# qiskit-community/adapt-aqc

Hardware: AMD Instinct MI355X
Metric: overlap+gradient evals/sec, 50-qubit MPS chi=64, 1/2/4/8 MI355X (higher is better)
Workload: dtype c128

## Files before the change

adaptaqc_amd/_lib.py:

```python
import atexit
import ctypes
import os
import threading

import numpy as np

_HERE = os.path.dirname(os.path.abspath(__file__))
LIB_PATH = os.environ.get("AQC_LIB") or os.path.join(_HERE, "libaqchip.so")

OP_DTYPE = np.dtype(
    [("nq", "<i4"), ("q0", "<i4"), ("q1", "<i4"), ("flags", "<i4"), ("m", "<f8", (32,))], align=True
)
assert OP_DTYPE.itemsize == 272
OP_KRAUS1 = 1
OP_MEASURE1 = 2
OP_KRAUS2 = 3

EXPORTS = (
    "aqc_last_error", "aqc_version", "aqc_init", "aqc_finalize", "aqc_timing_enable",
    "aqc_timing_query", "aqc_timing_reset",
    "aqc_sv_create", "aqc_sv_destroy", "aqc_sv_reset", "aqc_sv_copy", "aqc_sv_apply", "aqc_sv_plan",
    "aqc_sv_amp0", "aqc_sv_z_all", "aqc_sv_get", "aqc_sv_set",
    "aqc_mps_create", "aqc_mps_destroy", "aqc_mps_set_truncation", "aqc_mps_set_vidal",
    "aqc_mps_get_vidal", "aqc_mps_get_dims", "aqc_mps_copy", "aqc_mps_copy_batch", "aqc_mps_apply",
    "aqc_mps_apply_batch", "aqc_mps_apply_sort_batch", "aqc_mps_apply_sort_batch_async", "aqc_mps_apply_batch_async", "aqc_mps_check_batch", "aqc_mps_sort", "aqc_mps_sort_batch", "aqc_mps_overlap_zero",
    "aqc_mps_overlap_zero_batch", "aqc_mps_dot", "aqc_mps_z_all", "aqc_mps_amps_hw1", "aqc_mps_z_all_batch", "aqc_mps_z_sum_batch", "aqc_mps_zero_hw1_batch",
    "aqc_mps_amps_hw1_batch",
    "aqc_pair_grads", "aqc_pair_grads_batch", "aqc_argmax_scaled", "aqc_argmax_scaled_batch", "aqc_mps_jacobi_stats",
    "aqc_mps_set_jacobi_tol", "aqc_mps_set_jacobi_stop", "aqc_mps_set_fused_chain", "aqc_mps_chain_ticks", "aqc_svd_debug",
    "aqc_sv_pair_rdms", "aqc_mps_pair_rdms", "aqc_mps_pair_rdms_batch", "aqc_entanglement_measures",
    "aqc_sv_transition", "aqc_mps_product_fit", "aqc_mps_set_svd_path", "aqc_svd_gram_ticks", "aqc_bj_ticks",
    "aqc_sweep_set_chain_mode", "aqc_stream_join", "aqc_stream_wait", "aqc_svd_gram_stats", "aqc_env_ticks",
    "aqc_comm_unique_id", "aqc_comm_init", "aqc_comm_destroy", "aqc_comm_rank", "aqc_allgather_f64",
    "aqc_allgather_f64_host", "aqc_allreduce_max_f64", "aqc_svd_gram_big_stats", "aqc_svd_gram_big_ticks",
    "aqc_gb_set_spin_limit", "aqc_gb_set_tail", "aqc_gb_set_stages", "aqc_debug_hog", "aqc_pool_stats",
    "aqc_scratch_stats",
    "aqc_env_fallbacks", "aqc_env_set_single", "aqc_env_set_spin_limit",
    "aqc_sv_sample", "aqc_mps_sample", "aqc_sample_uniforms", "aqc_sv_traj_sample",
    "aqc_sv_traj_pair_tomo", "aqc_sv_traj_pauli_counts", "aqc_mps_traj_sample", "aqc_mps_traj_plan", "aqc_mps_traj_set_batch",
    "aqc_mps_traj_pair_tomo", "aqc_mps_traj_tomo_plan", "aqc_mps_traj_set_readout_batch",
    "aqc_sv_pauli_expect", "aqc_mps_pauli_expect", "aqc_mps_pauli_expect_batch",
    "aqc_pair_tomo_probs", "aqc_concurrence_bound_probs", "aqc_multinomial_counts", "aqc_tomo_fit",
)


class AqcError(RuntimeError):
    pass


_lock = threading.Lock()
_lib = None
_initialised_device = None

_P = ctypes.c_void_p
_I = ctypes.c_int
_D = ctypes.c_double
_DP = ctypes.POINTER(ctypes.c_double)
_IP = ctypes.POINTER(ctypes.c_int)

_SIGS = {
    "aqc_last_error": ([], ctypes.c_char_p),
    "aqc_version": ([], _I),
    "aqc_init": ([_I], _I),
    "aqc_finalize": ([], _I),
    "aqc_timing_enable": ([_I], _I),
    "aqc_timing_query": ([ctypes.c_char_p, _DP, ctypes.POINTER(ctypes.c_int64), _DP, _DP], _I),
    "aqc_timing_reset": ([], _I),
    "aqc_sv_create": ([_I, ctypes.POINTER(_P)], _I),
    "aqc_sv_destroy": ([_P], _I),
# ... 9 lines not shown
    "aqc_mps_destroy": ([_P], _I),
    "aqc_mps_set_truncation": ([_P, _D, _I], _I),
    "aqc_mps_set_vidal": ([_P, _P, _P, _P], _I),
    "aqc_mps_get_vidal": ([_P, _P, _P, _P], _I),
    "aqc_mps_get_dims": ([_P, _P], _I),
    "aqc_mps_copy": ([_P, _P], _I),
    "aqc_mps_copy_batch": ([_P, _P, _I], _I),
    "aqc_mps_apply": ([_P, _P, _I], _I),
    "aqc_mps_apply_batch": ([_P, _I, _P, _P], _I),
    "aqc_mps_apply_sort_batch": ([_P, _I, _P, _P], _I),
    "aqc_mps_apply_sort_batch_async": ([_P, _I, _P, _P], _I),
    "aqc_mps_apply_batch_async": ([_P, _I, _P, _P], _I),
    "aqc_mps_check_batch": ([_P, _I], _I),
    "aqc_mps_sort": ([_P], _I),
    "aqc_mps_sort_batch": ([_P, _I], _I),
    "aqc_mps_overlap_zero": ([_P, _DP, _DP], _I),
    "aqc_mps_overlap_zero_batch": ([_P, _I, _P], _I),
    "aqc_mps_dot": ([_P, _P, _DP, _DP], _I),
    "aqc_mps_z_all": ([_P, _P], _I),
    "aqc_mps_amps_hw1": ([_P, _P], _I),
    "aqc_mps_z_all_batch": ([_P, _I, _P], _I),
    "aqc_mps_z_sum_batch": ([_P, _P, _I, _P], _I),
    "aqc_mps_zero_hw1_batch": ([_P, _P, _I, _P, _P], _I),
    "aqc_mps_amps_hw1_batch": ([_P, _I, _P], _I),
    "aqc_pair_grads": ([_P, _P, _P, _I, _P, _P, _P, _I, _P, _I], _I),
    "aqc_pair_grads_batch": ([_P, _I, _P, _P, _I, _P, _P, _P, _I, _P, _I], _I),
    "aqc_argmax_scaled": ([_P, _P, _I, _I, _IP], _I),
    "aqc_argmax_scaled_batch": ([_P, _I, _P, _I, _I, _P], _I),
    "aqc_mps_jacobi_stats": ([_P, _IP], _I),
    "aqc_mps_set_jacobi_tol": ([_D], _I),
    "aqc_mps_set_jacobi_stop": ([_D], _I),
    "aqc_mps_set_fused_chain": ([_I], _I),
    "aqc_mps_chain_ticks": ([_P], _I),
    "aqc_svd_debug": ([_P, _I, _I, _I, _I, _P, _P, _P, _P], _I),
    "aqc_sv_pair_rdms": ([_P, _P, _I, _P], _I),
    "aqc_mps_pair_rdms": ([_P, _P, _I, _P], _I),
    "aqc_mps_pair_rdms_batch": ([_P, _I, _P, _I, _P, _I], _I),
    "aqc_entanglement_measures": ([_P, _I, _I, _P, _I], _I),
    "aqc_sv_transition": ([_P, _P, _I, _P], _I),
    "aqc_mps_product_fit": ([_P, _P, _I, _I, _I, _D, _DP, _IP], _I),
    "aqc_mps_set_svd_path": ([_I, _I], _I),
    "aqc_svd_gram_ticks": ([_P], _I),
    "aqc_bj_ticks": ([_P], _I),
    "aqc_sweep_set_chain_mode": ([_I], _I),
    "aqc_stream_join": ([_P], _I),
    "aqc_stream_wait": ([_P], _I),
    "aqc_svd_gram_stats": ([_P], _I),
    "aqc_env_ticks": ([_P], _I),
    "aqc_comm_unique_id": ([ctypes.c_char_p], _I),
    "aqc_comm_init": ([ctypes.c_char_p, _I, _I, ctypes.POINTER(_P)], _I),
    "aqc_comm_destroy": ([_P], _I),
    "aqc_comm_rank": ([_P, _IP, _IP], _I),
    "aqc_allgather_f64": ([_P, _P, _P, ctypes.c_size_t], _I),
    "aqc_allgather_f64_host": ([_P, _P, _P, ctypes.c_size_t], _I),
    "aqc_allreduce_max_f64": ([_P, _DP], _I),
    "aqc_svd_gram_big_stats": ([_P], _I),
    "aqc_svd_gram_big_ticks": ([_P], _I),
    "aqc_gb_set_spin_limit": ([_D], _I),
    "aqc_env_fallbacks": ([ctypes.POINTER(ctypes.c_longlong)], _I),
    "aqc_env_set_single": ([_I], _I),
    "aqc_env_set_spin_limit": ([_D], _I),
    "aqc_gb_set_tail": ([_I], _I),
    "aqc_gb_set_stages": ([_I], _I),
    "aqc_debug_hog": ([_I, _D], _I),
    "aqc_pool_stats": ([_P], _I),
    "aqc_scratch_stats": ([_P], _I),
# ... 94 lines not shown
    arr["q0"] = np.fromiter((q[0] for _, q in ops), dtype=np.int32, count=n)
    arr["q1"] = np.fromiter((q[1] if len(q) == 2 else 0 for _, q in ops), dtype=np.int32, count=n)
    m = arr["m"]
    for k, width in ((1, 4), (2, 16)):
        idx = np.flatnonzero(nq == k)
        if idx.size:
            mats = np.asarray([ops[i][0] for i in idx], dtype=np.complex128).reshape(idx.size, width)
            m[idx, : 2 * width] = mats.view(np.float64)
    return arr


def timing_enable(on=True):
    check(load().aqc_timing_enable(1 if on else 0))


def timing_reset():
    check(load().aqc_timing_reset())


def timing_query(name):
    ms, b, f = ctypes.c_double(), ctypes.c_double(), ctypes.c_double()
    n = ctypes.c_int64()
    check(load().aqc_timing_query(name.encode(), ctypes.byref(ms), ctypes.byref(n), ctypes.byref(b), ctypes.byref(f)))
    return {"ms": ms.value, "launches": n.value, "bytes": b.value, "flops": f.value}


def gram_stats():
    out = np.zeros(6)
    check(load().aqc_svd_gram_stats(ptr(out)))
    return {"calls": int(out[0]), "taken": int(out[1]), "declined_shape": int(out[2]),
            "declined_floor": int(out[3]), "certificates": int(out[4]), "certified": int(out[5])}


def gram_big_stats():
    out = np.zeros(8)
    check(load().aqc_svd_gram_big_stats(ptr(out)))
    return {"calls": int(out[0]), "taken": int(out[1]), "declined": int(out[2]),
            "declined_floor": int(out[3]), "timeouts": int(out[4]), "certificates": int(out[5]),
            "certified": int(out[6]), "declined_certificate": int(out[7])}
```

adaptaqc_amd/csrc/mps.hip:

```cpp
#include <algorithm>
#include <cmath>
#include <chrono>
#include <cstring>
#include <atomic>
#include <cstdlib>
#include <mutex>
#include <thread>
#include <unordered_set>

#include "aqc_gemm.h"
#include "mps_internal.h"

using aqc::cplx;

namespace aqc {

namespace {
std::mutex g_mps_stream_mu;
hipStream_t g_mps_streams[64] = {nullptr};
void release_mps_streams() {
  std::lock_guard<std::mutex> lk(g_mps_stream_mu);
  for (auto& s : g_mps_streams)
    if (s) (void)hipStreamDestroy(s), s = nullptr;
}
// ... 10 lines not shown
  }
  return g_mps_streams[dev];
}

hipStream_t mps_stream_if_any(int dev) {
  if (dev < 0 || dev >= 64) return nullptr;
  std::lock_guard<std::mutex> lk(g_mps_stream_mu);
  return g_mps_streams[dev];
}

StagingRing& staging_ring() {
  static PerDevice<StagingRing> rings;
  return rings.here();
}

}

namespace {

using aqc::fresh_tid;
using aqc::StagingLease;
using aqc::wave_sum_d;

constexpr int kT = 256;
constexpr double kChop = 1e-16;
constexpr int kMaxSweeps = 60;
double g_jacobi_tol_factor = 1.0;
constexpr double kDefaultTinyT = 1e-6;
constexpr double kStopCos = 3e-13;
constexpr int kStopCosSweeps = 30;
double g_jacobi_tiny_t = kDefaultTinyT;
constexpr double kJacobiNoise = 0.0;
bool g_fused_chain = true;
int g_chain_min_states = 32;
constexpr int kChainLdsBytes = 4 * (int)sizeof(aqc::GemmLds);

struct OneSiteJob {
  cplx* g;
  const int* dims;
  int cap;
  int pad;
  cplx u[4];
};

using aqc::TwoSiteJob;
using aqc::kMaxCap;
using aqc::kSigMax;
using aqc::kSigTail;
using aqc::kSigLen;

__global__ void k_mps_zero(cplx* gam, double* lam, int* dims, int n, int cap) {
  const size_t ss = (size_t)2 * cap * cap;
  for (int i = blockIdx.x * blockDim.x + threadIdx.x; i < n; i += gridDim.x * blockDim.x) {
    gam[(size_t)i * ss] = aqc::cmk(1.0, 0.0);
  }
  for (int b = blockIdx.x * blockDim.x + threadIdx.x; b <= n; b += gridDim.x * blockDim.x) {
    lam[(size_t)b * cap] = 1.0;
    dims[b] = 1;
  }
}

__global__ __launch_bounds__(kT) void k_1q(const OneSiteJob* __restrict__ jobs) {
  const OneSiteJob& j = jobs[blockIdx.y];
  const int cl = j.dims[0], cr = j.dims[1];
  const int cap = j.cap;
  const size_t half = (size_t)cap * cap;
// ... 580 lines not shown
  __shared__ double norm_s;
  const int chl = j.dims[0], chr = j.dims[2];
  const int M = 2 * chl, N = 2 * chr;
  const int C = M < N ? M : N;
  int P = 1;
  while (P < C) P <<= 1;
  const int tid = fresh_tid();
  for (int i = tid; i < P; i += NT) {
    sv[i] = i < C ? aqc::ldg(j.sig + i) : -1.0;
    si[i] = i;
  }
  __syncthreads();
  for (int k = 2; k <= P; k <<= 1) {
    for (int s = k >> 1; s > 0; s >>= 1) {
      for (int i = tid; i < P; i += NT) {
        const int ixj = i ^ s;
        if (ixj > i) {
          const bool desc = (i & k) == 0;
          const double a = sv[i], b = sv[ixj];
          const bool a_first = (a > b) || (a == b && si[i] < si[ixj]);
          if (a_first != desc) {
            sv[i] = b;
            sv[ixj] = a;
            const int t = si[i];
            si[i] = si[ixj];
            si[ixj] = t;
          }
        }
      }
      __syncthreads();
    }
  }
  if (tid == 0) {
    int k = 0;
    for (int i = 0; i < C; ++i)
      if (sv[i] * sv[i] > kChop) ++k;
    if (k < 1) k = 1;
    if (j.max_chi > 0 && k > j.max_chi) k = j.max_chi;
    double tail = aqc::ldg(j.sig + kSigTail);
    while (k > 1 && tail + sv[k - 1] * sv[k - 1] < j.thr) {
      tail += sv[k - 1] * sv[k - 1];
      --k;
    }
    aqc::stg(j.sig + kSigTail, 0.0);
    if (k > j.cap) {
      k = j.cap;
      atomicOr(&j.flags[0], 1);
    }
    double nn = 0.0;
    for (int i = 0; i < k; ++i) nn += sv[i] * sv[i];
    kk_s = k;
    norm_s = sqrt(nn);
    *(__attribute__((address_space(1))) int*)(j.dims + 1) = k;
  }
  __syncthreads();
  const int k = kk_s;
  for (int i = tid; i < k; i += NT) {
    aqc::stg(j.lm + i, sv[i] / norm_s);
    *(__attribute__((address_space(1))) int*)(j.perm + i) = si[i];
    aqc::stg(j.sig + i + kSigMax, sv[i]);
  }
}

__global__ __launch_bounds__(kT) void k_rank(const TwoSiteJob* __restrict__ jobs) { rank_body<kT>(jobs[blockIdx.x]); }

__device__ __forceinline__ void split_copy_body(const TwoSiteJob& j, int start, int stride) {
  const int chl = j.dims[0], k = j.dims[1], chr = j.dims[2];
  const int M = 2 * chl, N = 2 * chr;
  const bool tr = (M < N) != (j.qr != 0);
  const int L = tr ? N : M;
  const int cap = j.cap;
  const size_t half = (size_t)cap * cap;
  const double* ss = j.sig + kSigMax;
  if (!tr) {
    for (int e = start; e < 2 * chl * k; e += stride) {
      const int kk = e % k, rr = e / k;
      const int s1 = rr / chl, l = rr % chl;
      const double d = aqc::ldg(ss + kk) * aqc::ldg(j.ll + l);
      const cplx w = aqc::ldg(j.work + (size_t)j.perm[kk] * L + rr);
      aqc::stg(j.gp + s1 * half + (size_t)l * cap + kk, d != 0.0 ? aqc::cscale(w, 1.0 / d) : aqc::cmk(0, 0));
    }
  } else {
    for (int e = start; e < 2 * chr * k; e += stride) {
      const int cc = e % N, kk = e / N;
      const int s2 = cc / chr, r = cc % chr;
// ... 255 lines not shown
          for (int s2 = 0; s2 < 2; ++s2) {
            cr[s1][s2] = __builtin_amdgcn_mfma_f64_16x16x4f64(x[s2].x, y[s1].x, cr[s1][s2], 0, 0, 0);
            cr[s1][s2] = __builtin_amdgcn_mfma_f64_16x16x4f64(-x[s2].y, y[s1].y, cr[s1][s2], 0, 0, 0);
            ci[s1][s2] = __builtin_amdgcn_mfma_f64_16x16x4f64(x[s2].x, y[s1].y, ci[s1][s2], 0, 0, 0);
            ci[s1][s2] = __builtin_amdgcn_mfma_f64_16x16x4f64(x[s2].y, y[s1].x, ci[s1][s2], 0, 0, 0);
          }
      }
    }
    if (more) stash((c + 1) & 1, na, nb);
    __syncthreads();
  }
  if (active) {
    const int l = l0 + li;
#pragma unroll
    for (int q = 0; q < 4; ++q) {
      const int r = r0 + lk + 4 * q;
      if (l < chl && r < chr) {
        const cplx p0 = aqc::cmk(cr[0][0][q], ci[0][0][q]), p1 = aqc::cmk(cr[0][1][q], ci[0][1][q]);
        const cplx p2 = aqc::cmk(cr[1][0][q], ci[1][0][q]), p3 = aqc::cmk(cr[1][1][q], ci[1][1][q]);
#pragma unroll
        for (int o = 0; o < 4; ++o) {
          cplx v = aqc::cmul(sG[o * 4 + 0], p0);
          v = aqc::cfma(sG[o * 4 + 1], p1, v);
          v = aqc::cfma(sG[o * 4 + 2], p2, v);
          v = aqc::cfma(sG[o * 4 + 3], p3, v);
          aqc::stg(j.theta + (size_t)((o & 1) * chr + r) * M + (o >> 1) * chl + l, v);
        }
      }
    }
  }
}

__device__ __noinline__ void chain_jacobi_fallback(const TwoSiteJob& j) { jacobi_reg_body<128, 8, 16>(j); }
__device__ __forceinline__ void chain_jacobi(const TwoSiteJob& j) {
  if (j.gram) {
    const int g = gram_svd_body(j);
    if (g == 1) return;
    __syncthreads();
    if (g == 2 && gram_certified(j)) return;
  }
  chain_jacobi_fallback(j);
}
__device__ __forceinline__ void chain_rank(const TwoSiteJob& j) { rank_body<1024, 128>(j); }
__device__ __forceinline__ void split_gemm_chain(const TwoSiteJob& j, int tid) {
  extern __shared__ double2 xbuf[];
  const int sg = tid >> 8, lt = tid & 255, blk = sg >> 1, h = sg & 1;
  const int chl = j.dims[0], k = j.dims[1], chr = j.dims[2];
  const int M = 2 * chl, N = 2 * chr;
  const bool tr = (M < N) != (j.qr != 0);
  const int L = tr ? N : M;
  const int cap = j.cap;
  const size_t half = (size_t)cap * cap;
  const double* ss = j.sig + kSigMax;
  const int rows = tr ? M : k, cols = tr ? k : N;
  const int r0 = tr ? 64 * blk : 0, c0 = tr ? 0 : 64 * blk;
  const bool active = r0 < rows && c0 < cols;
  const int mb = active ? min(64, rows - r0) : 64, nb = active ? min(64, cols - c0) : 64;
  const int kh = ((L + 1) / 2 + 15) & ~15, klo = h * kh;
  const cplx* W = j.work;
  const int* perm = j.perm;
  const cplx* th = j.theta;
  aqc::GemmLds& lds = reinterpret_cast<aqc::GemmLds*>(xbuf)[sg];
  aqc::d4_t cr[2][2], ci[2][2];
  if (!tr) {
    aqc::block_cgemm_tile<true, true, false>(
        mb, nb, kh, 0, 0,
        [&](int kk, int R) {
          return klo + R < L ? aqc::cconj(aqc::ldg(W + (size_t)perm[r0 + kk] * L + klo + R)) : aqc::cmk(0, 0);
        },
        [&](int R, int c) { return klo + R < L ? aqc::ldg(th + (size_t)(c0 + c) * M + klo + R) : aqc::cmk(0, 0); }, lds, lt,
        active, cr, ci);
  } else {
    aqc::block_cgemm_tile<false, true, false>(
        mb, nb, kh, 0, 0,
// ... 8 lines not shown
#pragma unroll
    for (int r = 0; r < 2; ++r)
#pragma unroll
      for (int c = 0; c < 2; ++c)
#pragma unroll
        for (int q = 0; q < 4; ++q)
          part[(wr + 16 * r + lk + 4 * q) * 64 + wc + 16 * c + li] = aqc::cmk(cr[r][c][q], ci[r][c][q]);
  }
  __syncthreads();
  if (active && h == 0) {
#pragma unroll
    for (int r = 0; r < 2; ++r)
#pragma unroll
      for (int c = 0; c < 2; ++c)
#pragma unroll
        for (int q = 0; q < 4; ++q) {
          const int i = wr + 16 * r + lk + 4 * q, jj = wc + 16 * c + li;
          if (i < mb && jj < nb) {
            const cplx o = part[i * 64 + jj];
            const cplx v = aqc::cmk(cr[r][c][q] + o.x, ci[r][c][q] + o.y);
            if (!tr) {
              const int kq = r0 + i, cc = c0 + jj, s2 = cc / chr, rr = cc % chr;
              const double sk = aqc::ldg(ss + kq), d = sk * sk * aqc::ldg(j.lr + rr);
              aqc::stg(j.gq + s2 * half + (size_t)kq * cap + rr, d != 0.0 ? aqc::cscale(v, 1.0 / d) : aqc::cmk(0, 0));
            } else {
              const int Rr = r0 + i, kq = c0 + jj, s1 = Rr / chl, l = Rr % chl;
              const double sk = aqc::ldg(ss + kq), d = sk * sk * aqc::ldg(j.ll + l);
              aqc::stg(j.gp + s1 * half + (size_t)l * cap + kq, d != 0.0 ? aqc::cscale(v, 1.0 / d) : aqc::cmk(0, 0));
            }
          }
        }
  }
}
__device__ __forceinline__ void chain_split(const TwoSiteJob& j) {
  const int tid = fresh_tid();
  split_copy_body(j, tid, 1024);
  split_gemm_chain(j, tid);
}

__global__ __launch_bounds__(1024) void k_chain(const ChainJob* __restrict__ chains, const TwoSiteJob* __restrict__ two,
                                                const OneSiteJob* __restrict__ one) {
  const ChainJob& c = chains[blockIdx.x];
  const int tid = fresh_tid();
  __shared__ unsigned long long tk[6];
  if (tid == 0) tk[0] = tk[1] = tk[2] = tk[3] = tk[4] = tk[5] = 0;
  auto tick = [&](int ph) {
    if (tid == 0) {
      const unsigned long long t = __builtin_amdgcn_s_memtime();
      if (ph >= 0) tk[ph] += t - tk[5];
      tk[5] = t;
    }
  };
  tick(-1);
  for (int o = 0; o < c.nops; ++o) {
    const int code = __builtin_amdgcn_readfirstlane(c.ops[o]);
    if (code < 0) {
      one_site_body(one[-code - 1], tid, 1024);
      __syncthreads();
      tick(4);
      continue;
    }
    const TwoSiteJob& j = two[code];
#if AQC_THETA_MFMA
    chain_theta_mfma(j);
#else
    chain_theta(j);
#endif
    __syncthreads();
    tick(0);
    chain_jacobi(j);
    __syncthreads();
    tick(1);
    chain_rank(j);
    __syncthreads();
    tick(2);
    chain_split(j);
    __syncthreads();
    tick(3);
  }
  if (tid == 0)
    for (int ph = 0; ph < 5; ++ph) atomicAdd(&g_chain_ticks[ph], tk[ph]);
}

using aqc::DevOp;
using aqc::Scheduler;
using aqc::KrausJob;
using aqc::TrajCtx;
using aqc::run_waves;

template <class F>
void parallel_states(int ns, F&& f) {
  static const int kThreads = [] {
    const char* e = std::getenv("AQC_HOST_THREADS");
    const int v = e ? std::atoi(e) : 1;
    return v < 1 ? 1 : (v > 64 ? 64 : v);
  }();
  const int nt = std::min(kThreads, ns / 32);
  if (nt <= 1) {
    for (int s = 0; s < ns; ++s) f(s);
    return;
  }
  std::vector<std::thread> th;
  th.reserve(nt - 1);
  for (int t = 1; t < nt; ++t)
    th.emplace_back([&f, t, nt, ns] {
      for (int s = t; s < ns; s += nt) f(s);
    });
  for (int s = 0; s < ns; s += nt) f(s);
  for (auto& x : th) x.join();
// ... 137 lines not shown
  char* hb = sg.host;
  char* db = sg.dev;
  TwoSiteJob* h2 = (TwoSiteJob*)(hb + o_two);
  OneSiteJob* h1 = (OneSiteJob*)(hb + o_one);
  int* hcode = (int*)(hb + o_codes);
  parallel_states(ns, [&](int s) {
    size_t i2 = off2[s], i1 = off1[s], ic = offc[s];
    for (const DevOp& op : lists[s]) {
      if (op.kind == 2) {
        h2[i2] = make_two(hs[s], op, 0);
        h2[i2].qr = 1;
        hcode[ic++] = (int)i2++;
        std::vector<int>& ub = hs[s]->ub;
        int nb = std::min(2 * std::min(ub[op.p], ub[op.p + 2]), hs[s]->d.cap);
        if (hs[s]->max_chi > 0) nb = std::min(nb, hs[s]->max_chi);
        ub[op.p + 1] = std::max(nb, 1);
      } else {
        h1[i1] = make_one(hs[s], op);
        hcode[ic++] = -(int)(++i1);
      }
    }
  });
  ChainJob* hc = (ChainJob*)(hb + o_chain);
  for (int k = 0; k < ns; ++k) {
    const int s = order[k];
    hc[k].ops = (const int*)(db + o_codes) + offc[s];
    hc[k].nops = (int)lists[s].size();
    hc[k].pad = 0;
  }
  if (int e = aqc::upload_async(sg.dev, sg.host, total, st)) return e;
  const double c = cap_max, nj = (double)n_two;
  aqc::KernelTimer::begin(st, "mps_chain", nj * 8.0 * c * c * 16, nj * (84.0 * 8.0 + 64.0) * c * c * c);
  hipLaunchKernelGGL(k_chain, dim3(ns), dim3(1024), kChainLds, st, (const ChainJob*)(db + o_chain),
                     (const TwoSiteJob*)(db + o_two), (const OneSiteJob*)(db + o_one));
  aqc::KernelTimer::end(st);
  AQC_CHECK_LAUNCH();
  return AQC_OK;
}

KrausJob make_kraus(aqc_mps_t h, const DevOp& op, int shot) {
  KrausJob j;
  std::memset(&j, 0, sizeof(j));
  j.g = h->d.site(op.p);
  j.ll = h->d.bond(op.p);
  j.lr = h->d.bond(op.p + 1);
  j.dims = h->d.dims + op.p;
  j.cap = h->d.cap;
  j.nk = op.nk;
  j.slot = op.slot;
  j.meas = op.meas;
  j.shot = shot;
  std::memcpy(j.K, op.m, sizeof(j.K));
  for (int k = 0; k < op.nk; ++k) {
    const cplx* K = op.m + 4 * k;
    j.w[4 * k] = K[0].x * K[0].x + K[0].y * K[0].y + K[2].x * K[2].x + K[2].y * K[2].y;
    j.w[4 * k + 1] = K[1].x * K[1].x + K[1].y * K[1].y + K[3].x * K[3].x + K[3].y * K[3].y;
    j.w[4 * k + 2] = K[0].x * K[1].x + K[0].y * K[1].y + K[2].x * K[3].x + K[2].y * K[3].y;
    j.w[4 * k + 3] = K[0].x * K[1].y - K[0].y * K[1].x + K[2].x * K[3].y - K[2].y * K[3].x;
  }
  return j;
}

}

int aqc::run_waves(aqc_mps_t* hs, int ns, std::vector<std::vector<DevOp>>& lists, const TrajCtx* ctx) {
  bool kraus = false;
  for (int s = 0; s < ns; ++s) {
// ... 438 lines not shown
  unsigned long long t[6];
  AQC_HIP_CHECK(hipMemcpyFromSymbol(t, HIP_SYMBOL(g_gram_stats), sizeof(t)));
  for (int i = 0; i < 6; ++i) out[i] = (double)t[i];
  unsigned long long z[6] = {0, 0, 0, 0, 0, 0};
  AQC_HIP_CHECK(hipMemcpyToSymbol(HIP_SYMBOL(g_gram_stats), z, sizeof(z)));
  return AQC_OK;
}

int aqc_mps_set_svd_path(int gram, int debug_max_chi) {
  AQC_REQUIRE(gram >= 0 && gram <= 1, "aqc_mps_set_svd_path: gram must be 0 or 1");
  g_svd_gram = gram;
  g_debug_max_chi = debug_max_chi;
  return AQC_OK;
}


int aqc_mps_set_jacobi_stop(double tiny_t) {
  AQC_REQUIRE(tiny_t < 1e-3, "aqc_mps_set_jacobi_stop: tiny_t must be < 1e-3 (<= 0 restores the default)");
  g_jacobi_tiny_t = tiny_t > 0 ? tiny_t : kDefaultTinyT;
  return AQC_OK;
}

int aqc_mps_chain_ticks(double* out) {
  AQC_REQUIRE(out, "aqc_mps_chain_ticks: null argument");
  unsigned long long t[5] = {0, 0, 0, 0, 0};
  AQC_HIP_CHECK(hipStreamSynchronize(aqc::mps_stream()));
  AQC_HIP_CHECK(hipMemcpyFromSymbol(t, HIP_SYMBOL(g_chain_ticks), sizeof(t)));
  const unsigned long long z[5] = {0, 0, 0, 0, 0};
  AQC_HIP_CHECK(hipMemcpyToSymbol(HIP_SYMBOL(g_chain_ticks), z, sizeof(z)));
  for (int i = 0; i < 5; ++i) out[i] = (double)t[i];
  return AQC_OK;
}

int aqc_mps_set_fused_chain(int on) {
  AQC_REQUIRE(on >= 0 && on <= 2, "aqc_mps_set_fused_chain: 0, 1 or 2");
  g_fused_chain = on != 0;
  g_chain_min_states = on == 2 ? 1 : 32;
  return AQC_OK;
}


int aqc_mps_set_truncation(aqc_mps_t h, double threshold, int max_chi) {
  AQC_REQUIRE(h, "aqc_mps_set_truncation: null handle");
  h->thr = threshold;
  h->max_chi = max_chi;
  return AQC_OK;
}

int aqc_mps_set_vidal(aqc_mps_t h, const int* dims, const double* gammas, const double* lambdas) {
  AQC_REQUIRE(h && dims && gammas && lambdas, "aqc_mps_set_vidal: null argument");
  const int n = h->d.n, cap = h->d.cap;
  AQC_REQUIRE(dims[0] == 1 && dims[n] == 1, "aqc_mps_set_vidal: dims[0] and dims[n] must be 1");
  for (int b = 0; b <= n; ++b) {
    if (dims[b] < 1 || dims[b] > cap) {
      aqc::set_error("aqc_mps_set_vidal: bond dimension exceeds chi_cap");
      return AQC_ERR_ARG;
    }
  }
  std::vector<cplx> g((size_t)n * 2 * cap * cap, aqc::cmk(0, 0));
  std::vector<double> l((size_t)(n + 1) * cap, 0.0);
  size_t off = 0;
  for (int i = 0; i < n; ++i)
    for (int s = 0; s < 2; ++s)
      for (int a = 0; a < dims[i]; ++a)
        for (int b = 0; b < dims[i + 1]; ++b, ++off)
          g[(size_t)i * 2 * cap * cap + (size_t)s * cap * cap + (size_t)a * cap + b] =
// ... 253 lines not shown
```

adaptaqc_amd/csrc/svd_gram.h:

```cpp
#pragma once

constexpr int kGramMaxK = 128;
constexpr int kGramNarrowK = 64;
constexpr double kGramRelFloor = 1e-9;
__device__ unsigned long long g_gram_ticks[12];
static_assert(kGramNarrowK == 64, "S5: the narrow inverse iteration (tid < K) stays on wave 0");
__device__ unsigned long long g_gram_stats[6];

__device__ __forceinline__ double wave_sum_dpp(double v) {
  v = aqc::row_sum16(v);
  double s = 0.0;
#pragma unroll
  for (int rr = 0; rr < 4; ++rr) {
    const int lo = __builtin_amdgcn_readlane(__double2loint(v), 16 * rr);
    const int hi = __builtin_amdgcn_readlane(__double2hiint(v), 16 * rr);
    s += __hiloint2double(hi, lo);
  }
  return s;
}

__device__ __forceinline__ cplx pick16(const cplx (&g)[16], int i) {
  switch (i) {
#define AQC_PICK(n) \
  case n:           \
    return g[n];
    AQC_PICK(0) AQC_PICK(1) AQC_PICK(2) AQC_PICK(3) AQC_PICK(4) AQC_PICK(5) AQC_PICK(6) AQC_PICK(7)
    AQC_PICK(8) AQC_PICK(9) AQC_PICK(10) AQC_PICK(11) AQC_PICK(12) AQC_PICK(13) AQC_PICK(14)
#undef AQC_PICK
    default:
      return g[15];
  }
}

__device__ __forceinline__ double uniform_d(double v) {
  const int lo = __builtin_amdgcn_readfirstlane(__double2loint(v));
  const int hi = __builtin_amdgcn_readfirstlane(__double2hiint(v));
  return __hiloint2double(hi, lo);
}

__device__ __forceinline__ double bcast_d(double v, int l) {
// ... 171 lines not shown
      normalise(i);
    }
  }
}

template <int ZS>
__device__ __forceinline__ double rayleigh(int i, int C, const double* zb, const double* s_d, const double* s_e) {
  double s2a = 0.0, s2b = 0.0;
  int r0 = 0;
  constexpr int U = 8;
  for (; r0 + U <= C; r0 += U) {
    double zz[U + 1], dd[U], ee[U];
#pragma unroll
    for (int u = 0; u <= U; ++u) zz[u] = zb[min(r0 + u, C - 1) * ZS + i];
#pragma unroll
    for (int u = 0; u < U; ++u) dd[u] = s_d[r0 + u], ee[u] = r0 + u < C - 1 ? s_e[r0 + u] : 0.0;
#pragma unroll
    for (int u = 0; u < U; ++u) {
      s2a = fma(dd[u] * zz[u], zz[u], s2a);
      s2b = fma(2.0 * ee[u] * zz[u], zz[u + 1], s2b);
    }
  }
  for (; r0 < C; ++r0) {
    const double z = zb[r0 * ZS + i];
    s2a = fma(s_d[r0] * z, z, s2a);
    if (r0 < C - 1) s2b = fma(2.0 * s_e[r0] * z, zb[(r0 + 1) * ZS + i], s2b);
  }
  const double s2 = s2a + s2b;
  return s2 > 0.0 ? s2 : 0.0;
}

__device__ __forceinline__ void s6_back(const TwoSiteJob& j, cplx* hh, int C, int K, int c0, aqc::d4_t (&vre)[2],
                                        aqc::d4_t (&vim)[2], const double* s_sig2, int tid, int lane, int wave,
                                        int wave_s) {
  extern __shared__ double2 xbuf[];
  const int nt = wave & 3, mg = wave >> 2, li = lane & 15, lk = lane >> 4;
  cplx* Yl = xbuf;
  cplx* Pw = Yl + 2048;
  cplx* Tl = Pw + 12 * 256;
  cplx* W2l = Tl + 3 * 256 + 16 * 64;
  auto fetch_y = [&](int k0, int nb, cplx (&y)[2]) {
#pragma unroll
    for (int u = 0; u < 2; ++u) {
      const int e = tid + 1024 * u, row = e >> 4, i = e & 15, k = k0 + i;
      y[u] = (i < nb && row > k && row < C) ? aqc::ldg(hh + (size_t)k * (2 * C - k - 1) / 2 + (row - k - 1))
                                            : aqc::cmk(0, 0);
    }
  };
  cplx ynx[2];
  {
    const int k1 = C - 1, k0 = k1 > 16 ? k1 - 16 : 0;
    fetch_y(k0, k1 - k0, ynx);
  }
  __syncthreads();
  for (int k1 = C - 1; k1 > 0; k1 -= 16) {
    const int k0 = k1 > 16 ? k1 - 16 : 0;
#pragma unroll
    for (int u = 0; u < 2; ++u) {
      const int e = tid + 1024 * u, row = e >> 4, i = e & 15;
      Yl[row * 16 + (i ^ (row & 15))] = ynx[u];
    }
    if (tid < 256) {
      const gdbl_t* tp = (const gdbl_t*)(const double*)(hh + kTfacOff + (size_t)((C - 1 - k1) >> 4) * 512 + 256 + tid);
      Tl[(tid >> 4) * 17 + (tid & 15)] = aqc::cmk(__hip_atomic_load(tp, __ATOMIC_RELAXED, __HIP_MEMORY_SCOPE_AGENT),
                                                  __hip_atomic_load(tp + 1, __ATOMIC_RELAXED, __HIP_MEMORY_SCOPE_AGENT));
    }
    __syncthreads();
// ... 49 lines not shown
    }
    const int vl_ = fresh_lane();
    const int vmg = wave_s >> 2, vnt = wave_s & 3, vli = vl_ & 15, vlk = vl_ >> 4;
#pragma unroll
    for (int t = 0; t < 2; ++t) {
      if (32 * vmg + 16 * t + 15 > k0) {
        const int row = 32 * vmg + 16 * t + vli;
        aqc::d4_t p1 = {0, 0, 0, 0}, p2 = {0, 0, 0, 0};
#pragma unroll
        for (int s = 0; s < 4; ++s) {
          const int b = 4 * s + vlk;
          const cplx y = Yl[row * 16 + (b ^ (row & 15))];
          const cplx w = W2l[b * 64 + 16 * vnt + vli];
          p1 = __builtin_amdgcn_mfma_f64_16x16x4f64(y.x, w.x, p1, 0, 0, 0);
          p2 = __builtin_amdgcn_mfma_f64_16x16x4f64(y.y, w.y, p2, 0, 0, 0);
          vim[t] = __builtin_amdgcn_mfma_f64_16x16x4f64(-(y.x + y.y), w.x + w.y, vim[t], 0, 0, 0);
        }
#pragma unroll
        for (int q = 0; q < 4; ++q) vre[t][q] += p2[q] - p1[q], vim[t][q] += p1[q] + p2[q];
      }
    }
    __syncthreads();
  }
  {
    const int col = c0 + 16 * nt + li;
    if (col < K) {
      const double sg = sqrt(s_sig2[col]);
#pragma unroll
      for (int t = 0; t < 2; ++t) {
#pragma unroll
        for (int q = 0; q < 4; ++q) {
          const int row = 32 * mg + 16 * t + lk + 4 * q;
          if (row < C) aqc::stg(j.work + (size_t)col * C + row, aqc::cmk(vre[t][q] * sg, vim[t][q] * sg));
        }
      }
    }
  }
}

__device__ __noinline__ void s5_wide(int i, int C, const double* s_d, const double* s_e, const double* s_e2,
                                     double lam, double tn, double* zb, double* Db) {
  for (int row = 0; row < C; ++row) {
    unsigned int h = (unsigned int)(row * 2654435761u) ^ (unsigned int)((i + 1) * 40503u);
    h ^= h >> 13;
    h *= 0x5bd1e995u;
    h ^= h >> 15;
    zb[row * 128 + i] = (double)(h & 0xFFFFFu) * (2.0 / 1048576.0) - 1.0;
  }
  auto ldd = [&](int row) {
    return __hip_atomic_load((const gdbl_t*)(Db + row * 128 + i), __ATOMIC_RELAXED, __HIP_MEMORY_SCOPE_AGENT);
  };
  constexpr int U = 8;
  const double itn = 1.0 / fmax(tn, 1e-300), lamn = lam * itn;
  {
    double p0 = 0.0, p1 = 1.0;
    for (int row = 0; row < C; ++row) {
      const double d = s_d[row], e2 = s_e2[max(row - 1, 0)];
      const double dmx = fma(d, itn, -lamn), t = (e2 * itn * itn) * p0;
      const double lim = 2.220446049250313e-16 * fabs(p1);
      double p = fma(dmx, p1, -t);
      p = fabs(p) < lim ? copysign(lim, p) : p;
      aqc::stg(Db + row * 128 + i, p1 * rcp_nr(p) * itn);
      p0 = p1;
      p1 = p;
      if ((row & 7) == 7) {
        const int ex = max(__builtin_amdgcn_frexp_exp(p0), __builtin_amdgcn_frexp_exp(p1));
// ... 250 lines not shown
      acc.x += __shfl_xor(acc.x, 1);
      acc.y += __shfl_xor(acc.y, 1);
      const cplx p = rr > kk ? aqc::cmul(tau, acc) : aqc::cmk(0, 0);
      const double ktx = wave_sum_dpp(h == 0 ? fma(p.x, v.x, p.y * v.y) : 0.0);
      const double kty = wave_sum_dpp(h == 0 ? fma(p.x, v.y, -p.y * v.x) : 0.0);
      const cplx a2 = aqc::cscale(aqc::cmul(tau, aqc::cmk(ktx, kty)), -0.5);
      if (h == 0) pt[rr] = p;
      __builtin_amdgcn_fence(__ATOMIC_RELEASE, "workgroup");
      const double a2r2 = 2.0 * a2.x;
      const cplx w = aqc::cmk(fma(a2r2, v.x, p.x), fma(a2r2, v.y, p.y));
#pragma unroll
      for (int i = 0; i < 16; ++i) {
        if (2 * i + 1 > kk) {
          const cplx pc = pt[2 * i + h], vci = vt[2 * i + h];
          g[i].x = fma(-v.x, pc.x, fma(-v.y, pc.y, fma(-w.x, vci.x, fma(-w.y, vci.y, g[i].x))));
          g[i].y = fma(-v.y, pc.x, fma(v.x, pc.y, fma(-w.y, vci.x, fma(w.x, vci.y, g[i].y))));
        }
      }
    }
    const cplx glast = pick16(g, (kS3Tail - 1) >> 1);
    const double dl = bcast_d(glast.x, 2 * (kS3Tail - 1) + ((kS3Tail - 1) & 1));
    if (lane == 0) dS[C - 1] = dl;
  }
}

#ifndef AQC_GRAM_INLINE
#define AQC_GRAM_INLINE 0
#endif
#if AQC_GRAM_INLINE
__device__ __forceinline__
#else
__device__ __noinline__
#endif
int gram_svd_body(const TwoSiteJob& j) {
  extern __shared__ double2 xbuf[];
  __shared__ double s_d[128], s_e[128], s_e2[128], s_lam[128], s_err[128], s_sig2[kGramMaxK], s_tail;
  __shared__ int s_K, s_cert;
  __shared__ cplx s_tau[128];
  __shared__ double s_lo, s_hi, s_tn;
  __shared__ double2 s_de[128];
  const int chl = j.dims[0], chr = j.dims[2];
  const int M = 2 * chl, N = 2 * chr;
  const bool tr = M < N;
  const int L = tr ? N : M, C = tr ? M : N;
  const int KE = (j.max_chi > 0 && j.max_chi < C) ? j.max_chi : C;
  const int tid = fresh_tid(), lane = tid & 63, wave = tid >> 6;
  const int wave_s = __builtin_amdgcn_readfirstlane(wave);
  if (tid == 0) atomicAdd(&g_gram_stats[0], 1ull);
  if (C < 4 || C > 128 || L > 128 || j.cap < 64) {
    if (tid == 0) atomicAdd(&g_gram_stats[2], 1ull);
    return 0;
  }
  const cplx* th = j.theta;
  unsigned long long t_last = tid == 0 ? __builtin_amdgcn_s_memtime() : 0ull;
  auto tick = [&](int ph) {
    if (tid == 0) {
      const unsigned long long t = __builtin_amdgcn_s_memtime();
      atomicAdd(&g_gram_ticks[ph], t - t_last);
      t_last = t;
    }
  };
  unsigned long long t_a = 0, t_b = 0;
  auto tick_step = [&](unsigned long long& acc) {
    if (tid == 0) {
      const unsigned long long t = __builtin_amdgcn_s_memtime();
      acc += t - t_last;
      t_last = t;
    }
  };
  const int r0 = tid >> 3, q0 = tid & 7;
// ... 472 lines not shown
      int r0 = 0;
      for (; r0 + U <= C; r0 += U) {
        double zz[U];
#pragma unroll
        for (int u = 0; u < U; ++u) zz[u] = zb[(r0 + u) * 64 + i];
#pragma unroll
        for (int u = 0; u < U; ++u) zb[(r0 + u) * 64 + i] = zz[u] * sc;
      }
      for (; r0 < C; ++r0) zb[r0 * 64 + i] *= sc;
    }
    if (tid == 0) atomicAdd(&g_gram_ticks[7], __builtin_amdgcn_s_memtime() - t_last);
  }
  else if ((wave & 3) != 0 && wave - 1 - (wave >> 2) < ((C - 1 + 15) >> 4)) {
    s6_factors(wave - 1 - (wave >> 2), C, hh, s_tau, lane);
  }
  __syncthreads();
  if (wave == 0)
    gs_clusters<64>(K, C, zb, s_lam, s_e, s_tn, lane, [&](int row, int i) { return Db[row * 64 + i]; });
  __syncthreads();
  if (tid < K) s_sig2[tid] = rayleigh<64>(tid, C, zb, s_d, s_e);
  __syncthreads();
  tick(3);
  const int nt = wave & 3, mg = wave >> 2, li = lane & 15, lk = lane >> 4;
  aqc::d4_t vre[2], vim[2];
#pragma unroll
  for (int t = 0; t < 2; ++t) {
#pragma unroll
    for (int q = 0; q < 4; ++q) {
      const int row = 32 * mg + 16 * t + lk + 4 * q, col = 16 * nt + li;
      vre[t][q] = (row < C && col < K) ? zb[row * 64 + col] : 0.0;
      vim[t][q] = 0.0;
    }
  }
  s6_back(j, hh, C, K, 0, vre, vim, s_sig2, tid, lane, wave, wave_s);
  tick(4);
  }
  for (int c = tid; c < C; c += 1024) aqc::stg(j.sig + c, c < K ? sqrt(s_sig2[c]) : 0.0);
  if (tid == 0) aqc::stg(j.sig + kSigTail, s_tail);
  tick(5);
  if (s_cert) return 2;
  if (tid == 0) {
    atomicMax(&j.flags[2], 1);
    atomicAdd(&g_gram_stats[1], 1ull);
  }
  return 1;
}

__device__ __noinline__ bool gram_certified(const TwoSiteJob& j) {
  const int tid = fresh_tid();
  __shared__ double s_s2[128];
  __shared__ int s_k;
  const int M = 2 * j.dims[0], N = 2 * j.dims[2], C = M < N ? M : N;
  if (tid == 0) s_k = 0;
  __syncthreads();
  if (tid < C) {
    const double sg = aqc::ldg(j.sig + tid);
    s_s2[tid] = sg * sg;
    if (sg > 0.0) atomicMax(&s_k, tid + 1);
  }
  __syncthreads();
  if (tid == 0) atomicAdd(&g_gram_stats[4], 1ull);
  const double cs = gram_cert128(j, C, s_k, s_s2);
  const bool ok = cs < 0.5 * aqc::kReduceChop;
  if (tid == 0) {
    atomicAdd(&g_gram_stats[ok ? 5 : 3], 1ull);
    if (ok) {
      atomicMax(&j.flags[2], 1);
      atomicAdd(&g_gram_stats[1], 1ull);
    } else {
      aqc::stg(j.sig + kSigTail, 0.0);
    }
  }
  __syncthreads();
  return ok;
}

__global__ __launch_bounds__(1024) void k_svd_gram(const TwoSiteJob* __restrict__ jobs) {
  const TwoSiteJob& j = jobs[blockIdx.x];
  const int g = j.gram ? gram_svd_body(j) : 0;
  if (g == 1) return;
  __syncthreads();
  if (g == 2 && gram_certified(j)) return;
  jacobi_reg_body<128, 8, 16>(j);
}
```

include/aqc_hip_diag.h:

```cpp
#ifndef AQC_HIP_DIAG_H
#define AQC_HIP_DIAG_H

#include "aqc_hip.h"

#ifdef __cplusplus
extern "C" {
#endif

int aqc_mps_jacobi_stats(aqc_mps_t h, int* max_sweeps);
int aqc_mps_set_jacobi_tol(double factor);
int aqc_mps_set_jacobi_stop(double tiny_t);
int aqc_mps_set_svd_path(int gram, int debug_max_chi);
int aqc_svd_gram_ticks(double* out);
int aqc_svd_gram_stats(double* out);
int aqc_env_ticks(double* out);
int aqc_env_fallbacks(long long* out);
int aqc_env_set_single(int on);
int aqc_env_set_spin_limit(double us);
int aqc_bj_ticks(double* out);
int aqc_svd_gram_big_stats(double* out);
int aqc_svd_gram_big_ticks(double* out);
int aqc_gb_set_spin_limit(double us);
int aqc_gb_set_tail(int on);
int aqc_gb_set_stages(int n);
int aqc_debug_hog(int nblocks, double ms);
int aqc_pool_stats(double* out);
int aqc_scratch_stats(double* out);
int aqc_mps_set_fused_chain(int on);
int aqc_mps_chain_ticks(double* out);
int aqc_svd_debug(const double* theta, int m, int n, int variant, int stop_after_qr, double* w_out,
                  double* sig_out, int* perm_out, int* sweeps);
int aqc_sweep_set_chain_mode(int mode);
int aqc_sample_uniforms(uint64_t seed, uint64_t run, int nshots, int nper, double* out);
#ifdef __cplusplus
}
#endif
#endif
```

Baseline: 8.078 million.

## Fuse rank selection and split copy into gram SVD epilogue of chain kernel

Inside the fused chain kernel, the gram SVD body can now decide the truncation rank itself when its singular values are already sorted. It writes lambda, perm and sigma directly and skips the separate rank_body pass. In mode 2 it also writes the scaled gamma factors during back-transformation, so the split copy pass is skipped too. The rank rule is moved into a shared helper, and the new behaviour is selectable by environment variable or API, with mode 1 as the default. This adds per-lane stores and branching in the SVD epilogue, and uses a different sorting check that falls back when values are unsorted.

```diff
diff --git a/adaptaqc_amd/_lib.py b/adaptaqc_amd/_lib.py
--- a/adaptaqc_amd/_lib.py
+++ b/adaptaqc_amd/_lib.py
@@ -34,7 +34,7 @@
     "aqc_comm_unique_id", "aqc_comm_init", "aqc_comm_destroy", "aqc_comm_rank", "aqc_allgather_f64",
     "aqc_allgather_f64_host", "aqc_allreduce_max_f64", "aqc_svd_gram_big_stats", "aqc_svd_gram_big_ticks",
     "aqc_gb_set_spin_limit", "aqc_gb_set_tail", "aqc_gb_set_stages", "aqc_debug_hog", "aqc_pool_stats",
-    "aqc_scratch_stats",
+    "aqc_scratch_stats", "aqc_mps_set_chain_epilogue", "aqc_mps_chain_epilogue_stats",
     "aqc_env_fallbacks", "aqc_env_set_single", "aqc_env_set_spin_limit",
     "aqc_sv_sample", "aqc_mps_sample", "aqc_sample_uniforms", "aqc_sv_traj_sample",
     "aqc_sv_traj_pair_tomo", "aqc_sv_traj_pauli_counts", "aqc_mps_traj_sample", "aqc_mps_traj_plan", "aqc_mps_traj_set_batch",
@@ -110,6 +110,8 @@
     "aqc_mps_set_jacobi_stop": ([_D], _I),
     "aqc_mps_set_fused_chain": ([_I], _I),
     "aqc_mps_chain_ticks": ([_P], _I),
+    "aqc_mps_set_chain_epilogue": ([_I], _I),
+    "aqc_mps_chain_epilogue_stats": ([_P], _I),
     "aqc_svd_debug": ([_P, _I, _I, _I, _I, _P, _P, _P, _P], _I),
     "aqc_sv_pair_rdms": ([_P, _P, _I, _P], _I),
     "aqc_mps_pair_rdms": ([_P, _P, _I, _P], _I),
@@ -270,6 +272,12 @@
             "declined_floor": int(out[3]), "certificates": int(out[4]), "certified": int(out[5])}
 
 
+def chain_epilogue_stats():
+    out = np.zeros(2)
+    check(load().aqc_mps_chain_epilogue_stats(ptr(out)))
+    return {"fused": int(out[0]), "unsorted": int(out[1])}
+
+
 def gram_big_stats():
     out = np.zeros(8)
     check(load().aqc_svd_gram_big_stats(ptr(out)))
diff --git a/adaptaqc_amd/csrc/mps.hip b/adaptaqc_amd/csrc/mps.hip
--- a/adaptaqc_amd/csrc/mps.hip
+++ b/adaptaqc_amd/csrc/mps.hip
@@ -66,6 +66,11 @@
 double g_jacobi_tiny_t = kDefaultTinyT;
 constexpr double kJacobiNoise = 0.0;
 bool g_fused_chain = true;
+int g_chain_epilogue = [] {
+  const char* e = std::getenv("AQC_CHAIN_EPILOGUE");
+  const int v = e ? std::atoi(e) : 1;
+  return v >= 0 && v <= 2 ? v : 1;
+}();
 int g_chain_min_states = 32;
 constexpr int kChainLdsBytes = 4 * (int)sizeof(aqc::GemmLds);
 
@@ -712,25 +717,11 @@
     }
   }
   if (tid == 0) {
-    int k = 0;
-    for (int i = 0; i < C; ++i)
-      if (sv[i] * sv[i] > kChop) ++k;
-    if (k < 1) k = 1;
-    if (j.max_chi > 0 && k > j.max_chi) k = j.max_chi;
-    double tail = aqc::ldg(j.sig + kSigTail);
-    while (k > 1 && tail + sv[k - 1] * sv[k - 1] < j.thr) {
-      tail += sv[k - 1] * sv[k - 1];
-      --k;
-    }
+    double nrm;
+    const int k = rank_rule(j, sv, C, aqc::ldg(j.sig + kSigTail), nrm);
     aqc::stg(j.sig + kSigTail, 0.0);
-    if (k > j.cap) {
-      k = j.cap;
-      atomicOr(&j.flags[0], 1);
-    }
-    double nn = 0.0;
-    for (int i = 0; i < k; ++i) nn += sv[i] * sv[i];
     kk_s = k;
-    norm_s = sqrt(nn);
+    norm_s = nrm;
     *(__attribute__((address_space(1))) int*)(j.dims + 1) = k;
   }
   __syncthreads();
@@ -1052,14 +1043,16 @@
 }
 
 __device__ __noinline__ void chain_jacobi_fallback(const TwoSiteJob& j) { jacobi_reg_body<128, 8, 16>(j); }
-__device__ __forceinline__ void chain_jacobi(const TwoSiteJob& j) {
+__device__ __forceinline__ int chain_jacobi(const TwoSiteJob& j, int epi) {
   if (j.gram) {
-    const int g = gram_svd_body(j);
-    if (g == 1) return;
+    const int g = gram_svd_body(j, epi);
+    if (g == 1) return 0;
+    if (g > 2) return g - 2;
     __syncthreads();
-    if (g == 2 && gram_certified(j)) return;
+    if (g == 2 && gram_certified(j)) return 0;
   }
   chain_jacobi_fallback(j);
+  return 0;
 }
 __device__ __forceinline__ void chain_rank(const TwoSiteJob& j) { rank_body<1024, 128>(j); }
 __device__ __forceinline__ void split_gemm_chain(const TwoSiteJob& j, int tid) {
@@ -1134,14 +1127,14 @@
         }
   }
 }
-__device__ __forceinline__ void chain_split(const TwoSiteJob& j) {
+__device__ __forceinline__ void chain_split(const TwoSiteJob& j, bool copied) {
   const int tid = fresh_tid();
-  split_copy_body(j, tid, 1024);
+  if (!copied) split_copy_body(j, tid, 1024);
   split_gemm_chain(j, tid);
 }
 
 __global__ __launch_bounds__(1024) void k_chain(const ChainJob* __restrict__ chains, const TwoSiteJob* __restrict__ two,
-                                                const OneSiteJob* __restrict__ one) {
+                                                const OneSiteJob* __restrict__ one, int epi) {
   const ChainJob& c = chains[blockIdx.x];
   const int tid = fresh_tid();
   __shared__ unsigned long long tk[6];
@@ -1170,13 +1163,13 @@
 #endif
     __syncthreads();
     tick(0);
-    chain_jacobi(j);
+    const int done = __builtin_amdgcn_readfirstlane(chain_jacobi(j, epi));
     __syncthreads();
     tick(1);
-    chain_rank(j);
+    if (done == 0) chain_rank(j);
     __syncthreads();
     tick(2);
-    chain_split(j);
+    chain_split(j, done == 2);
     __syncthreads();
     tick(3);
   }
@@ -1380,7 +1373,7 @@
   const double c = cap_max, nj = (double)n_two;
   aqc::KernelTimer::begin(st, "mps_chain", nj * 8.0 * c * c * 16, nj * (84.0 * 8.0 + 64.0) * c * c * c);
   hipLaunchKernelGGL(k_chain, dim3(ns), dim3(1024), kChainLds, st, (const ChainJob*)(db + o_chain),
-                     (const TwoSiteJob*)(db + o_two), (const OneSiteJob*)(db + o_one));
+                     (const TwoSiteJob*)(db + o_two), (const OneSiteJob*)(db + o_one), g_chain_epilogue);
   aqc::KernelTimer::end(st);
   AQC_CHECK_LAUNCH();
   return AQC_OK;
@@ -1885,6 +1878,23 @@
   return AQC_OK;
 }
 
+int aqc_mps_set_chain_epilogue(int mode) {
+  AQC_REQUIRE(mode >= 0 && mode <= 2, "aqc_mps_set_chain_epilogue: 0, 1 or 2");
+  g_chain_epilogue = mode;
+  return AQC_OK;
+}
+
+int aqc_mps_chain_epilogue_stats(double* out) {
+  AQC_REQUIRE(out, "aqc_mps_chain_epilogue_stats: null argument");
+  unsigned long long t[2] = {0, 0};
+  AQC_HIP_CHECK(hipStreamSynchronize(aqc::mps_stream()));
+  AQC_HIP_CHECK(hipMemcpyFromSymbol(t, HIP_SYMBOL(g_epi_stats), sizeof(t)));
+  const unsigned long long z[2] = {0, 0};
+  AQC_HIP_CHECK(hipMemcpyToSymbol(HIP_SYMBOL(g_epi_stats), z, sizeof(z)));
+  for (int i = 0; i < 2; ++i) out[i] = (double)t[i];
+  return AQC_OK;
+}
+
 int aqc_mps_set_fused_chain(int on) {
   AQC_REQUIRE(on >= 0 && on <= 2, "aqc_mps_set_fused_chain: 0, 1 or 2");
   g_fused_chain = on != 0;
diff --git a/adaptaqc_amd/csrc/svd_gram.h b/adaptaqc_amd/csrc/svd_gram.h
--- a/adaptaqc_amd/csrc/svd_gram.h
+++ b/adaptaqc_amd/csrc/svd_gram.h
@@ -6,6 +6,27 @@
 __device__ unsigned long long g_gram_ticks[12];
 static_assert(kGramNarrowK == 64, "S5: the narrow inverse iteration (tid < K) stays on wave 0");
 __device__ unsigned long long g_gram_stats[6];
+__device__ unsigned long long g_epi_stats[2];
+
+__device__ __forceinline__ int rank_rule(const TwoSiteJob& j, const double* sv, int n, double tail, double& norm) {
+  int k = 0;
+  for (int i = 0; i < n; ++i)
+    if (sv[i] * sv[i] > kChop) ++k;
+  if (k < 1) k = 1;
+  if (j.max_chi > 0 && k > j.max_chi) k = j.max_chi;
+  while (k > 1 && tail + sv[k - 1] * sv[k - 1] < j.thr) {
+    tail += sv[k - 1] * sv[k - 1];
+    --k;
+  }
+  if (k > j.cap) {
+    k = j.cap;
+    atomicOr(&j.flags[0], 1);
+  }
+  double nn = 0.0;
+  for (int i = 0; i < k; ++i) nn += sv[i] * sv[i];
+  norm = sqrt(nn);
+  return k;
+}
 
 __device__ __forceinline__ double wave_sum_dpp(double v) {
   v = aqc::row_sum16(v);
@@ -243,7 +264,7 @@
 
 __device__ __forceinline__ void s6_back(const TwoSiteJob& j, cplx* hh, int C, int K, int c0, aqc::d4_t (&vre)[2],
                                         aqc::d4_t (&vim)[2], const double* s_sig2, int tid, int lane, int wave,
-                                        int wave_s) {
+                                        int wave_s, bool copy = false, bool gtr = false, const int* s_fk = nullptr) {
   extern __shared__ double2 xbuf[];
   const int nt = wave & 3, mg = wave >> 2, li = lane & 15, lk = lane >> 4;
   cplx* Yl = xbuf;
@@ -359,6 +380,28 @@
         for (int q = 0; q < 4; ++q) {
           const int row = 32 * mg + 16 * t + lk + 4 * q;
           if (row < C) aqc::stg(j.work + (size_t)col * C + row, aqc::cmk(vre[t][q] * sg, vim[t][q] * sg));
+        }
+      }
+    }
+    if (copy && col < *s_fk) {
+      const int chs = C >> 1;
+      const size_t half = (size_t)j.cap * j.cap;
+      const double sg = sqrt(s_sig2[col]);
+      const double* lo = gtr ? j.ll : j.lr;
+#pragma unroll
+      for (int t = 0; t < 2; ++t) {
+#pragma unroll
+        for (int q = 0; q < 4; ++q) {
+          const int row = 32 * mg + 16 * t + lk + 4 * q;
+          if (row < C) {
+            const int s = row >= chs, o = row - s * chs;
+            const double d = sg * aqc::ldg(lo + o);
+            cplx w = aqc::cmk(vre[t][q] * sg, vim[t][q] * sg);
+            if (!gtr) w = aqc::cconj(w);
+            w = d != 0.0 ? aqc::cscale(w, 1.0 / d) : aqc::cmk(0, 0);
+            if (gtr) aqc::stg(j.gp + s * half + (size_t)o * j.cap + col, w);
+            else aqc::stg(j.gq + s * half + (size_t)col * j.cap + o, w);
+          }
         }
       }
     }
@@ -675,10 +718,10 @@
 #else
 __device__ __noinline__
 #endif
-int gram_svd_body(const TwoSiteJob& j) {
+int gram_svd_body(const TwoSiteJob& j, int epi) {
   extern __shared__ double2 xbuf[];
   __shared__ double s_d[128], s_e[128], s_e2[128], s_lam[128], s_err[128], s_sig2[kGramMaxK], s_tail;
-  __shared__ int s_K, s_cert;
+  __shared__ int s_K, s_cert, s_fk;
   __shared__ cplx s_tau[128];
   __shared__ double s_lo, s_hi, s_tn;
   __shared__ double2 s_de[128];
@@ -1217,18 +1260,43 @@
       vim[t][q] = 0.0;
     }
   }
-  s6_back(j, hh, C, K, 0, vre, vim, s_sig2, tid, lane, wave, wave_s);
+  if (epi == 2 && j.qr == 0) epi = 1;
+  if (epi && !s_cert && wave == 0) {
+    const double sg = lane < K ? sqrt(s_sig2[lane]) : 0.0;
+    s_err[lane] = sg;
+    const bool ok = __ballot(lane >= K - 1 || sg >= __shfl_down(sg, 1)) == ~0ull;
+    __builtin_amdgcn_wave_barrier();
+    double nrm = 0.0;
+    int k = 0;
+    if (lane == 0) {
+      if (ok) {
+        k = rank_rule(j, s_err, K, s_tail, nrm);
+        *(__attribute__((address_space(1))) int*)(j.dims + 1) = k;
+      }
+      s_fk = k;
+      atomicAdd(&g_epi_stats[ok ? 0 : 1], 1ull);
+    }
+    k = __builtin_amdgcn_readfirstlane(k);
+    nrm = uniform_d(nrm);
+    if (lane < k) {
+      aqc::stg(j.lm + lane, sg / nrm);
+      *(__attribute__((address_space(1))) int*)(j.perm + lane) = lane;
+      aqc::stg(j.sig + lane + kSigMax, sg);
+    }
+  }
+  s6_back(j, hh, C, K, 0, vre, vim, s_sig2, tid, lane, wave, wave_s, epi == 2 && !s_cert, tr, &s_fk);
   tick(4);
   }
+  const int fk = (epi && !s_cert && K <= kGramNarrowK) ? __builtin_amdgcn_readfirstlane(s_fk) : 0;
   for (int c = tid; c < C; c += 1024) aqc::stg(j.sig + c, c < K ? sqrt(s_sig2[c]) : 0.0);
-  if (tid == 0) aqc::stg(j.sig + kSigTail, s_tail);
+  if (tid == 0) aqc::stg(j.sig + kSigTail, fk ? 0.0 : s_tail);
   tick(5);
   if (s_cert) return 2;
   if (tid == 0) {
     atomicMax(&j.flags[2], 1);
     atomicAdd(&g_gram_stats[1], 1ull);
   }
-  return 1;
+  return fk ? 2 + epi : 1;
 }
 
 __device__ __noinline__ bool gram_certified(const TwoSiteJob& j) {
@@ -1262,7 +1330,7 @@
 
 __global__ __launch_bounds__(1024) void k_svd_gram(const TwoSiteJob* __restrict__ jobs) {
   const TwoSiteJob& j = jobs[blockIdx.x];
-  const int g = j.gram ? gram_svd_body(j) : 0;
+  const int g = j.gram ? gram_svd_body(j, 0) : 0;
   if (g == 1) return;
   __syncthreads();
   if (g == 2 && gram_certified(j)) return;
diff --git a/include/aqc_hip_diag.h b/include/aqc_hip_diag.h
--- a/include/aqc_hip_diag.h
+++ b/include/aqc_hip_diag.h
@@ -27,6 +27,8 @@
 int aqc_pool_stats(double* out);
 int aqc_scratch_stats(double* out);
 int aqc_mps_set_fused_chain(int on);
+int aqc_mps_set_chain_epilogue(int mode);
+int aqc_mps_chain_epilogue_stats(double* out);
 int aqc_mps_chain_ticks(double* out);
 int aqc_svd_debug(const double* theta, int m, int n, int variant, int stop_after_qr, double* w_out,
                   double* sig_out, int* perm_out, int* sweeps);
```

After: 8.191 million, median of 6. 1.01x the previous value.
